# aproposorg/sydr

Measured on AMD Instinct MI355X. Metric: IQ Msamples/s through 32-ch E/P/L correlators @25 MHz fs, higher is better.
Workload: dtype f64

## Files before the change

sydr_amd/csrc/correlator_chip.h:

```cpp
#pragma once

#include "correlator.h"

#pragma clang fp contract(off)

namespace sdr {

constexpr int kChipMax = 26;
constexpr double kChipMinCodeStep = 1.0 / 25.9;
constexpr double kChipMaxCodeStep = 1.0 / 15.5;
constexpr int kChipRawDwords = 13;
constexpr int kChipRotSlots = 2 * kChipMax + 2;
template <int NT>
constexpr int chip_strip_slots() { return 2 * NT + 1; }

__host__ __device__ __forceinline__ int chip_first_above(double thr, double shift, double inv_step, bool& near) {
    const double u = (thr - shift) * inv_step;
    const double fl = floor(u);
    const double fr = u - fl;
    near = near || fr < kNearInteger || fr > 1.0 - kNearInteger;
    return (int)fl + 1;
}
__host__ __device__ __forceinline__ int chip_first_above_exact(int c, double thr, double step, double shift) {
    auto above = [&](int i) {
        double y = (double)i * step;
        y = y + shift;
        return y > thr;
    };
    if (c >= 1 && above(c - 1)) return (c >= 2 && above(c - 2)) ? c - 2 : c - 1;
    if (c < 0) c = 0;
    if (above(c)) return c;
    return above(c + 1) ? c + 1 : c + 2;
}

template <int B, int E, class F>
__device__ __forceinline__ void static_for(F&& f) {
    if constexpr (B < E) {
        f(std::integral_constant<int, B>{});
        static_for<B + 1, E>(f);
    }
}

__device__ __forceinline__ int wave_min_i32(int x) {
#pragma unroll
    for (int off = 1; off < 64; off <<= 1) {
        const int o = __shfl_xor(x, off, 64);
        x = o < x ? o : x;
    }
    return __builtin_amdgcn_readfirstlane(x);
}

#ifndef SDR_BIASED_CVT
#define SDR_BIASED_CVT 1
#endif
constexpr double kCvtBias = 4224.0;
typedef uint32_t sdr_u32x2 __attribute__((ext_vector_type(2)));
__device__ __forceinline__ double biased_sample(sdr_u32x2& pair, uint32_t w_flipped, uint32_t selector, uint32_t hi_const) {
    pair.y = __builtin_amdgcn_perm(w_flipped, hi_const, selector);
    return __builtin_bit_cast(double, pair);
}
constexpr uint32_t cvt_selector(int byte) { return 0x03020000u | ((uint32_t)(4 + byte) << 8) | 0x0Cu; }

template <int NT>
struct ChipGeom {
    int64_t Tfx, Ufx;
    uint64_t delta[NT];
    int q0, F;
    int head_end, tail_start;
    int m[NT], J[NT];
    int bad;
};

template <int NT, int KM, int KS, int KI>
__host__ __device__ __forceinline__ void chip_geometry(int n, const double* shift, const double* step, const double* inv_step,
                                                       ChipGeom<NT>& g) {
    constexpr int A = NT / 2;
    const double two32 = 4294967296.0;
    g.q0 = (int)ceil(shift[A]);
    double y_last = (double)(n - 1) * step[A];
    y_last = y_last + shift[A];
    const int q_last = (int)ceil(y_last);
    g.F = q_last - g.q0 - 1;
    g.head_end = n, g.tail_start = n;
    if (g.F > 0) {
        bool nr = false;
        g.head_end = chip_first_above_exact(chip_first_above((double)g.q0, shift[A], inv_step[A], nr), (double)g.q0, step[A], shift[A]);
        g.tail_start = chip_first_above_exact(chip_first_above((double)(q_last - 1), shift[A], inv_step[A], nr),
                                              (double)(q_last - 1), step[A], shift[A]);
    }
    g.Tfx = (int64_t)rint(inv_step[A] * two32);
    g.Ufx = (int64_t)floor(-shift[A] * inv_step[A] * two32);
    const int M = (int)(g.Tfx >> 32);
    bool bad = M < 1 || M + 1 > kChipMax || g.F > 16384 || (KM != 0 && M != KM);
#pragma unroll
    for (int t = 0; t < NT; ++t) {
        g.m[t] = M, g.J[t] = 0, g.delta[t] = 0;
        if (t == A) continue;
        const int64_t Ut = (int64_t)floor(-shift[t] * inv_step[t] * two32);
        int j = (int)ceil(shift[t] - shift[A]) - 1;
        int64_t d = (Ut - g.Ufx) + (int64_t)(1 + j) * g.Tfx;
        if (d < 0) {
            d += g.Tfx;
            ++j;
        } else if (d >= g.Tfx) {
            d -= g.Tfx;
            --j;
        }
        bad = bad || d < 0 || d >= g.Tfx;
        g.J[t] = j;
        g.delta[t] = (uint64_t)d;
        g.m[t] = (int)(d >> 32);
        bad = bad || (KS != 0 && (g.m[t] != KS || j != (t < A ? -1 : 0)));
        bad = bad || (KI != 0 && !((j == (t - A) * KI - 1 && g.m[t] == 0) || (j == (t - A) * KI && g.m[t] >= M)));
    }
    g.bad = bad ? 1 : 0;
}

constexpr int kStaticHalf = 13;
constexpr int chip_half(int KM, int KS, int KI) { return KI != 0 ? (KM + 2) / 2 : KS + 1; }
struct ChipRot {
    double urc[kStaticHalf + 1], urs[kStaticHalf + 1];
    double rd0c, rd0s, rd1c, rd1s;
    double biasc[3], biass[3];
};
__host__ __device__ inline void chip_rotations(double dphi, int Dmin, ChipRot& r, int half = kStaticHalf, int cmin = kStaticHalf - 2) {
    double cs[16], sn[16];
    for (int k = 0; k < 16; ++k) sincos_reduced(-(double)k * dphi, &sn[k], &cs[k]);
    for (int k = 1; k <= half; ++k) r.urc[k] = cs[k], r.urs[k] = sn[k];
    r.urc[0] = 1.0, r.urs[0] = 0.0;
    sincos_reduced(-(double)Dmin * dphi, &r.rd0s, &r.rd0c);
    sincos_reduced(-(double)(Dmin + 1) * dphi, &r.rd1s, &r.rd1c);
    for (int st = 1; st < 16; st <<= 1)
        for (int l = 15; l >= st; --l) cs[l] += cs[l - st], sn[l] += sn[l - st];
    for (int i = 0; i < 3; ++i) {
        const int l = cmin + i - 1;
        const double re = cs[l] - sn[l], im = cs[l] + sn[l];
        r.biasc[i] = re * 4224.0, r.biass[i] = im * 4224.0;
    }
}

template <int NT>
struct ChipSetup {
    double dphi;
    double shift[NT], step[NT], inv_step[NT];
    int64_t base;
    ChipGeom<NT> g;
    ChipRot r;
};

template <int NT, int KM, int KS, int KI>
__host__ __device__ inline void chip_setup(int n, int64_t start_sample, int64_t capacity, double carrier_hz, double rem_code,
                                           double code_step, const double* spacing, double fs, int stride, ChipSetup<NT>& S) {
    S = ChipSetup<NT>{};
    S.dphi = carrier_step(carrier_hz, fs);
    const double nd = (double)n;
    for (int t = 0; t < NT; ++t) {
        const double shift = rem_code + spacing[t];
        double stop = code_step * nd;
        stop = stop + shift;
        const double delta = stop - shift;
        S.shift[t] = shift;
        S.step[t] = delta / nd;
        S.inv_step[t] = 1.0 / S.step[t];
    }
    const int64_t base = start_sample % capacity;
    const bool applies = code_step >= kChipMinCodeStep && code_step <= kChipMaxCodeStep && base + n + 32 <= capacity;
    S.base = applies ? base : -1;
    if (applies) {
        chip_geometry<NT, KM, KS, KI>(n, S.shift, S.step, S.inv_step, S.g);
        chip_rotations(S.dphi, (int)(((int64_t)stride * S.g.Tfx) >> 32), S.r, chip_half(KM, KS, KI), KM - chip_half(KM, KS, KI));
    }
}

template <int NT>
struct ChipBlock {
    uint32_t raw[kChipRawDwords];
    int S;
    int dn;
    int ds[NT];
};

template <int NT, bool SINGLE_WAVE, int KM = 0, int KS = 0, int KI = 0>
__device__ __forceinline__ bool correlate_epoch_chip(const void* __restrict__ ring, const void* __restrict__ ring_flipped, int64_t capacity,
                                                     const EpochParams& ep, double dphi, const EpochConsts<NT>& K,
                                                     const ChipGeom<NT>& G, int64_t base, const ChipRot* R,
                                                     const uint32_t* lut, double2* strip_lds, double2* rot, int tid,
                                                     int lane, int stride, int edge_lane, double* accr, double* acci) {
    constexpr int A = NT / 2;
    constexpr int kSlots = chip_strip_slots<NT>();
    const int n = ep.n;
    const double* shift = K.shift;
    const double* step = K.step;
    double2* strip = strip_lds + tid * kSlots;
    const int wlane = threadIdx.x & 63;
#pragma unroll
    for (int t = 0; t < NT; ++t) accr[t] = acci[t] = 0.0;

    const double dphi_u = uniform(dphi), rem_carrier_u = uniform(ep.rem_carrier);
    const int q0 = __builtin_amdgcn_readfirstlane(G.q0);
    const int F = __builtin_amdgcn_readfirstlane(G.F);
    const int head_end = __builtin_amdgcn_readfirstlane(G.head_end);
    const int tail_start = __builtin_amdgcn_readfirstlane(G.tail_start);
    (void)ring_flipped;
    const char* ring_base = static_cast<const char*>(ring) + base * 2;

    static_assert(!(KS != 0 && KI != 0), "either the taps switch inside the block (KS) or with it (KI)");
    constexpr bool kStatic = KM != 0 && (KS != 0 || KI != 0);
    constexpr int kHalf = chip_half(KM, KS, KI);
    double urc[kStatic ? kHalf + 1 : 1], urs[kStatic ? kHalf + 1 : 1];
    double biasc[3] = {0.0, 0.0, 0.0}, biass[3] = {0.0, 0.0, 0.0};
    const double two32 = 4294967296.0;
    int64_t Tfx = G.Tfx;
    int64_t stride_fx = (int64_t)stride * Tfx;
    const int Dmin = (int)(stride_fx >> 32);
    if constexpr (kStatic) asm volatile("" : "+v"(Tfx), "+v"(stride_fx));
    double rd0c = 1.0, rd0s = 0.0, rd1c = 1.0, rd1s = 0.0;
    {
        double sn = 0.0, cs = 0.0;
        if constexpr (kStatic) {
            static_assert(kHalf <= kStaticHalf, "the plan's rotations are laid out for half blocks of up to 13 samples");
#pragma unroll
            for (int k = 1; k <= kHalf; ++k) urc[k] = R->urc[k], urs[k] = R->urs[k];
            rd0c = R->rd0c, rd0s = R->rd0s, rd1c = R->rd1c, rd1s = R->rd1s;
            if constexpr (SDR_BIASED_CVT) {
#pragma unroll
                for (int i = 0; i < 3; ++i) biasc[i] = R->biasc[i], biass[i] = R->biass[i];
            }
        } else {
            if (wlane < kChipMax) {
                sincos_reduced(-(double)wlane * dphi_u, &sn, &cs);
                rot[wlane] = make_double2(cs, sn);
            }
            if constexpr (SDR_BIASED_CVT) {
                double br = (cs - sn) * kCvtBias, bi = (cs + sn) * kCvtBias;
#pragma unroll
                for (int off = 1; off < 32; off <<= 1) {
                    const double o_r = __shfl_up(br, off, 64), o_i = __shfl_up(bi, off, 64);
                    br = wlane >= off ? br + o_r : br;
                    bi = wlane >= off ? bi + o_i : bi;
                }
                double2* const btab = rot + kChipMax;
                if (wlane < kChipMax) btab[wlane + 1] = make_double2(br, bi);
                if (wlane == 0) btab[0] = make_double2(0.0, 0.0);
            }
        }
    }

    bool bad = false;
    const int rounds = F > 0 ? (F + stride - 1) / stride : 0;
    if (rounds > 0) {
        int64_t Ufx = G.Ufx;
        const int M = (int)(G.Tfx >> 32);
        if constexpr (kStatic) asm volatile("" : "+v"(Ufx));
        bad = bad || G.bad != 0;
        int m[NT], J[NT];
        uint64_t delta[NT];
        unsigned evmask = (1u << M) | (2u << M);
#pragma unroll
        for (int t = 0; t < NT; ++t) {
            m[t] = G.m[t], J[t] = G.J[t], delta[t] = G.delta[t];
            if constexpr (kStatic) asm volatile("" : "+v"(m[t]), "+v"(J[t]), "+v"(delta[t]));
            if (t != A) evmask |= (1u << m[t]) | (2u << m[t]);
        }
        const int k_last = M + 1;
        int rank[NT];
#pragma unroll
        for (int t = 0; t < NT; ++t) rank[t] = __builtin_popcount(evmask & ((1u << m[t]) - 1u));
        if constexpr (!kStatic) {
            double sn, cs;
            sincos_reduced(-(double)(Dmin + (wlane & 1)) * dphi_u, &sn, &cs);
            rd0c = lane_value(cs, 0), rd0s = lane_value(sn, 0);
            rd1c = lane_value(cs, 1), rd1s = lane_value(sn, 1);
        }
        asm volatile("" : "+v"(rd0c), "+v"(rd0s), "+v"(rd1c), "+v"(rd1s));
        const uint64_t lane_fx = (uint64_t)((int64_t)lane * Tfx);
        uint64_t u_cur = (uint64_t)(Ufx + (int64_t)q0 * Tfx + (int64_t)two32) + lane_fx;
        const int last_idx = F - 1;

        auto prepare = [&](int round, uint64_t u0, ChipBlock<NT>& b) {
            const int idx = round * stride + lane;
            const bool inside = idx <= last_idx;
            const uint64_t uS = inside ? u0 : (uint64_t)(Ufx + (int64_t)(q0 + last_idx) * Tfx + (int64_t)two32);
            const uint64_t uE = uS + (uint64_t)Tfx;
            int S = (int)(uS >> 32);
            int E = (int)(uE >> 32);
            bool near = (uint32_t)uS + 0x10000u < 0x20000u || (uint32_t)uE + 0x10000u < 0x20000u;
            int split[NT];
#pragma unroll
            for (int t = 0; t < NT; ++t) {
                split[t] = 0;
                if (t == A) continue;
                if constexpr (KI != 0) {
                    split[t] = J[t] == (t - A) * KI ? E - S : 0;
                    continue;
                }
                const uint64_t uT = uS + delta[t];
                near = near || (uint32_t)uT + 0x10000u < 0x20000u;
                split[t] = (int)(uT >> 32) - S;
            }
            if (__builtin_expect(__any(near), 0)) {
                const int q = q0 + 1 + (inside ? idx : last_idx);
                S = chip_first_above_exact(S, (double)(q - 1), step[A], shift[A]);
                E = chip_first_above_exact(E, (double)q, step[A], shift[A]);
#pragma unroll
                for (int t = 0; t < NT; ++t) {
                    if (t == A) continue;
                    const int p0 = q + J[t];
                    const int bt = chip_first_above_exact(S + split[t], (double)p0, step[t], shift[t]);
                    double y = (double)S * step[t];
                    y = y + shift[t];
                    const int at_s = (int)ceil(y);
                    bad = bad || (at_s != p0 && at_s != p0 + 1) || (at_s == p0 + 1 && bt > S);
                    split[t] = bt < S ? 0 : bt - S;
                }
            }
            b.S = S;
            const int nn = E - S;
            b.dn = nn - M;
            bad = bad || (unsigned)b.dn > 1u;
#pragma unroll
            for (int t = 0; t < NT; ++t) {
                b.ds[t] = 0;
                if (t == A) continue;
                const int sp = split[t] > nn ? nn : split[t];
                if constexpr (KI != 0) {
                    bad = bad || !(J[t] == (t - A) * KI ? sp == nn : sp == 0);
                    continue;
                }
                b.ds[t] = sp - m[t];
                bad = bad || (unsigned)b.ds[t] > 1u;
            }
            if constexpr (KS != 0 && NT == 3) bad = bad || b.ds[0] != b.ds[2];
            const char* src = ring_base + (int64_t)S * 2;
            const uint4 w0 = *reinterpret_cast<const uint4*>(src);
            const uint4 w1 = *reinterpret_cast<const uint4*>(src + 16);
            const uint4 w2 = *reinterpret_cast<const uint4*>(src + 32);
            const uint32_t w3 = *reinterpret_cast<const uint32_t*>(src + 48);
            b.raw[0] = w0.x, b.raw[1] = w0.y, b.raw[2] = w0.z, b.raw[3] = w0.w;
            b.raw[4] = w1.x, b.raw[5] = w1.y, b.raw[6] = w1.z, b.raw[7] = w1.w;
            b.raw[8] = w2.x, b.raw[9] = w2.y, b.raw[10] = w2.z, b.raw[11] = w2.w;
            b.raw[12] = w3;
        };

        ChipBlock<NT> blk_a, blk_b;
        prepare(0, u_cur, blk_a);
        double sb, cb;
        sincos_reduced(__builtin_fma(-(double)blk_a.S, dphi_u, rem_carrier_u), &sb, &cb);
        if constexpr (!kStatic) {
            sb = lane <= last_idx ? sb : 0.0;
            cb = lane <= last_idx ? cb : 0.0;
        }
        const int q_lane = q0 + 1 + lane + SDR_LUT_PAD;
        const uint32_t* zero_lq = reinterpret_cast<const uint32_t*>(strip) + 3;
        if constexpr (kStatic) strip[0] = strip[1] = make_double2(0.0, 0.0);

        sdr_u32x2 zI = {0u, 0u}, zQ = {0u, 0u};
        asm volatile("" : "+v"(zI), "+v"(zQ));

        auto process = [&](const ChipBlock<NT>& b, int round, double sbk, double cbk) {
            double pr = 0.0, pi = 0.0;
            double2* wp = strip;
            unsigned evm = evmask;
            int klast = k_last;
            if constexpr (!kStatic) asm volatile("" : "+s"(evm), "+s"(klast));
            constexpr int kAhead = 4;
            double2 rr[kChipMax + kAhead];
            if constexpr (!kStatic) {
#pragma unroll
                for (int k = 0; k < kAhead; ++k) rr[k] = rot[k];
            }
            auto park = [&]() {
                *wp = make_double2(pr, pi);
                ++wp;
                asm volatile("" ::: "memory");
            };
            uint32_t hi_rt = 0x40B00000u;
            uint32_t sel_rt[4] = {cvt_selector(0), cvt_selector(1), cvt_selector(2), cvt_selector(3)};
            if constexpr (!kStatic && SDR_BIASED_CVT) {
                asm volatile("" : "+v"(hi_rt));
                asm volatile("" : "+s"(sel_rt[0]), "+s"(sel_rt[1]), "+s"(sel_rt[2]), "+s"(sel_rt[3]));
            }
            auto sample = [&](auto kc) {
                constexpr int k = decltype(kc)::value;
                double ar, ai;
                if constexpr (SDR_BIASED_CVT) {
                    ar = biased_sample(zI, b.raw[k >> 1], sel_rt[(k & 1) ? 2 : 0], hi_rt);
                    ai = biased_sample(zQ, b.raw[k >> 1], sel_rt[(k & 1) ? 3 : 1], hi_rt);
                } else {
                    const int w = ci8_native((int)b.raw[k >> 1]);
                    ar = (k & 1) ? (double)(int)(int8_t)(w >> 16) : (double)(int)(int8_t)w;
                    ai = (k & 1) ? (double)(w >> 24) : (double)(int)(int8_t)(w >> 8);
                }
                if (k + kAhead < kChipMax) rr[k + kAhead] = rot[k + kAhead];
                const double2 r = rr[k];
                pr = __builtin_fma(-ai, r.y, __builtin_fma(ar, r.x, pr));
                pi = __builtin_fma(ai, r.x, __builtin_fma(ar, r.y, pi));
                if constexpr (SDR_BIASED_CVT) asm volatile("" : "+v"(pr), "+v"(pi), "+v"(zI), "+v"(zQ));
            };
            double capr[3] = {0.0, 0.0, 0.0}, capi[3] = {0.0, 0.0, 0.0};
            if constexpr (kStatic) {
                static_assert(2 * kHalf >= KM + 1 && kHalf < KM, "two halves of at most KS + 1 samples cover the block");
                static_assert(!SDR_BIASED_CVT || (2 * kHalf - KM >= 1 && 2 * kHalf - KM <= 2 && (KS == 0 || KS == kHalf - 1)),
                              "the offset's shares are kept for sums of KM - kHalf, + 1 and + 2 samples: kHalf must be one of the last two");
                uint32_t flipped[kChipRawDwords];
                uint32_t hi_const = 0x40B00000u;
                if constexpr (SDR_BIASED_CVT) {
                    asm volatile("" : "+v"(hi_const));
#pragma unroll
                    for (int i = 0; i < kChipRawDwords; ++i) flipped[i] = b.raw[i];
                }
                static_for<0, KM + 1>([&](auto kc) {
                    constexpr int k = decltype(kc)::value;
                    constexpr int j = k < kHalf ? k : k - kHalf;
                    const int w = ci8_native((int)b.raw[k >> 1]);
                    double ar, ai;
                    if constexpr (SDR_BIASED_CVT) {
                        ar = biased_sample(zI, flipped[k >> 1], cvt_selector((k & 1) ? 2 : 0), hi_const);
                        ai = biased_sample(zQ, flipped[k >> 1], cvt_selector((k & 1) ? 3 : 1), hi_const);
                    } else {
                        ar = (k & 1) ? (double)(int)(int8_t)(w >> 16) : (double)(int)(int8_t)w;
                        ai = (k & 1) ? (double)(w >> 24) : (double)(int)(int8_t)(w >> 8);
                    }
                    if constexpr (KS != 0 && k == KS) capr[0] = pr, capi[0] = pi;
                    if constexpr (k == KM) capr[1] = pr, capi[1] = pi;
                    if constexpr (k == kHalf) capr[2] = pr, capi[2] = pi;
                    if constexpr (j == 0) {
                        pr = ar, pi = ai;
                    } else {
                        pr = __builtin_fma(-ai, urs[j], __builtin_fma(ar, urc[j], pr));
                        pi = __builtin_fma(ai, urc[j], __builtin_fma(ar, urs[j], pi));
                    }
                    if constexpr (SDR_BIASED_CVT) asm volatile("" : "+v"(pr), "+v"(pi), "+v"(zI), "+v"(zQ));
                });
            } else if constexpr (KM != 0) {
                static_for<0, KM>([&](auto kc) {
                    constexpr int k = decltype(kc)::value;
                    if (evm & (1u << k)) park();
                    sample(kc);
                });
                park();
                sample(std::integral_constant<int, KM>{});
                park();
            } else {
#pragma unroll
                for (int k = 0; k <= kChipMax; ++k) {
                    if (evm & (1u << k)) {
                        park();
                        if (k == klast) break;
                    }
                    if (k < kChipMax) {
                        double ar, ai;
                        if constexpr (SDR_BIASED_CVT) {
                            ar = biased_sample(zI, b.raw[k >> 1], sel_rt[(k & 1) ? 2 : 0], hi_rt);
                            ai = biased_sample(zQ, b.raw[k >> 1], sel_rt[(k & 1) ? 3 : 1], hi_rt);
                        } else {
                            const int w = ci8_native((int)b.raw[k >> 1]);
                            ar = (k & 1) ? (double)(int)(int8_t)(w >> 16) : (double)(int)(int8_t)w;
                            ai = (k & 1) ? (double)(w >> 24) : (double)(int)(int8_t)(w >> 8);
                        }
                        if (k + kAhead < kChipMax) rr[k + kAhead] = rot[k + kAhead];
                        const double2 r = rr[k];
                        pr = __builtin_fma(-ai, r.y, __builtin_fma(ar, r.x, pr));
                        pi = __builtin_fma(ai, r.x, __builtin_fma(ar, r.y, pi));
                        if constexpr (SDR_BIASED_CVT) asm volatile("" : "+v"(pr), "+v"(pi), "+v"(zI), "+v"(zQ));
                    }
                }
            }
            double2 ptot;
            if constexpr (kStatic && SDR_BIASED_CVT) {
                constexpr int iFirst = 2 * kHalf - KM;
                pr -= biasc[1], pi -= biass[1];
                capr[1] -= biasc[0], capi[1] -= biass[0];
                capr[2] -= biasc[iFirst], capi[2] -= biass[iFirst];
                if constexpr (KS != 0) capr[0] -= biasc[iFirst - 1], capi[0] -= biass[iFirst - 1];
            }
            if constexpr (kStatic) {
                const double qr = b.dn ? pr : capr[1], qi = b.dn ? pi : capi[1];
                ptot.x = __builtin_fma(-qi, urs[kHalf], __builtin_fma(qr, urc[kHalf], capr[2]));
                ptot.y = __builtin_fma(qi, urc[kHalf], __builtin_fma(qr, urs[kHalf], capi[2]));
            } else {
                ptot = strip[rank[A] + b.dn];
                if constexpr (SDR_BIASED_CVT) {
                    const double2 bb = (rot + kChipMax)[M + b.dn];
                    ptot.x -= bb.x, ptot.y -= bb.y;
                }
            }
            const int first = round * stride;
            const uint32_t* lq;
            if constexpr (kStatic)
                lq = first + lane <= last_idx ? lut + q_lane + first : zero_lq;
            else
                lq = lut + q_lane + (first + lane <= last_idx ? first : last_idx - lane);
            if constexpr (KI != 0) {
                const double xr = __builtin_fma(-sbk, ptot.y, cbk * ptot.x);
                const double xi = __builtin_fma(sbk, ptot.x, cbk * ptot.y);
#pragma unroll
                for (int t = 0; t < NT; ++t) {
                    const double c = __hiloint2double((int)lq[(t - A) * KI], 0);
                    accr[t] = __builtin_fma(c, xr, accr[t]);
                    acci[t] = __builtin_fma(c, xi, acci[t]);
                }
                return;
            }
#pragma unroll
            for (int t = 0; t < NT; ++t) {
                double gr, gi;
                if (t == A) {
                    const double c = __hiloint2double((int)lq[0], 0);
                    gr = c * ptot.x;
                    gi = c * ptot.y;
                } else {
                    double2 ps;
                    if constexpr (kStatic)
                        ps = b.ds[NT == 3 ? 0 : t] ? make_double2(capr[2], capi[2]) : make_double2(capr[0], capi[0]);
                    else {
                        ps = strip[rank[t] + b.ds[t]];
                        if constexpr (SDR_BIASED_CVT) {
                            const double2 bb = (rot + kChipMax)[m[t] + b.ds[t]];
                            ps.x -= bb.x, ps.y -= bb.y;
                        }
                    }
                    const int jt = kStatic ? (t < A ? -1 : 0) : J[t];
                    const double ca = __hiloint2double((int)lq[jt], 0);
                    const double cbn = __hiloint2double((int)lq[jt + 1], 0);
                    const double diff = ca - cbn;
                    gr = __builtin_fma(diff, ps.x, cbn * ptot.x);
                    gi = __builtin_fma(diff, ps.y, cbn * ptot.y);
                }
                accr[t] = __builtin_fma(-sbk, gi, __builtin_fma(cbk, gr, accr[t]));
                acci[t] = __builtin_fma(sbk, gr, __builtin_fma(cbk, gi, acci[t]));
            }
        };

        auto wave_has_work = [&](int round) { return SINGLE_WAVE || round * stride + (lane - wlane) <= last_idx; };
        auto advance = [&](const ChipBlock<NT>& from, const ChipBlock<NT>& to, int to_round) {
            const unsigned dd = (unsigned)(to.S - from.S - Dmin);
            const bool alive = to_round * stride + lane <= last_idx;
            bad = bad || (alive && dd > 1u);
            const double rc_ = dd ? rd1c : rd0c, rs_ = dd ? rd1s : rd0s;
            const double cbn = __builtin_fma(cb, rc_, -sb * rs_);
            const double sbn = __builtin_fma(sb, rc_, cb * rs_);
            if constexpr (kStatic) {
                cb = cbn, sb = sbn;
            } else {
                cb = alive ? cbn : 0.0;
                sb = alive ? sbn : 0.0;
            }
        };

        for (int it = 0; it < rounds / 2; ++it) {
            const double sb0 = sb, cb0 = cb;
            u_cur += (uint64_t)stride_fx;
            prepare(2 * it + 1, u_cur, blk_b);
            advance(blk_a, blk_b, 2 * it + 1);
            if (wave_has_work(2 * it)) process(blk_a, 2 * it, sb0, cb0);
            const double sb1 = sb, cb1 = cb;
            if (2 * it + 2 < rounds) {
                u_cur += (uint64_t)stride_fx;
                prepare(2 * it + 2, u_cur, blk_a);
                advance(blk_b, blk_a, 2 * it + 2);
            }
            if (wave_has_work(2 * it + 1)) process(blk_b, 2 * it + 1, sb1, cb1);
        }
        if ((rounds & 1) && wave_has_work(rounds - 1)) process(blk_a, rounds - 1, sb, cb);
    }

    if (__any(bad)) return false;
    if (edge_lane >= 0) {
        if (head_end + (n - tail_start) > 64) {
            for (int off = 0; off < head_end + (n - tail_start); off += 64)
                edge_samples<SDR_FMT_CI8, NT>(ring, capacity, ep, dphi, shift, step, lut, edge_lane + off, head_end, tail_start, accr, acci, base);
        } else {
            edge_samples<SDR_FMT_CI8, NT>(ring, capacity, ep, dphi, shift, step, lut, edge_lane, head_end, tail_start, accr, acci, base);
        }
    }
    return true;
}

__device__ __forceinline__ bool chip_variant_applies(const EpochParams& ep, int64_t capacity) {
    return ep.code_step >= kChipMinCodeStep && ep.code_step <= kChipMaxCodeStep &&
           ep.start_sample % capacity + ep.n + 32 <= capacity;
}

}
```

Before: 96730.

## Track chip block positions with 32-bit fractional walk and derive splits from carries

Replaces the per-block 64-bit fixed-point position arithmetic with a 32-bit fractional walker that advances by the stride and detects boundary crossings via carry bits. In the common case the block length and tap splits are derived directly from carry comparisons, and the exact slow path runs only when some lane is near a boundary. The phase advance now uses the walk carry instead of comparing block starts. It also relaxes a few asm register barriers in the biased conversion path. This cuts integer ALU and register pressure per block but adds ballot and popcount overhead plus more complex consistency checks.

```diff
diff --git a/sydr_amd/csrc/correlator_chip.h b/sydr_amd/csrc/correlator_chip.h
--- a/sydr_amd/csrc/correlator_chip.h
+++ b/sydr_amd/csrc/correlator_chip.h
@@ -114,6 +114,51 @@
         bad = bad || (KI != 0 && !((j == (t - A) * KI - 1 && g.m[t] == 0) || (j == (t - A) * KI && g.m[t] >= M)));
     }
     g.bad = bad ? 1 : 0;
+}
+
+template <int NT>
+struct ChipWalk {
+    uint32_t t_lo, stride_lo, delta_lo[NT];
+    int M, Dmin, m[NT];
+};
+struct ChipWalkPos {
+    int S;
+    uint32_t f;
+};
+template <int NT>
+__host__ __device__ __forceinline__ ChipWalk<NT> chip_walk_make(const ChipGeom<NT>& g, int stride) {
+    ChipWalk<NT> w;
+    const int64_t stride_fx = (int64_t)stride * g.Tfx;
+    w.t_lo = (uint32_t)g.Tfx, w.M = (int)(g.Tfx >> 32);
+    w.stride_lo = (uint32_t)stride_fx, w.Dmin = (int)(stride_fx >> 32);
+#pragma unroll
+    for (int t = 0; t < NT; ++t) w.delta_lo[t] = (uint32_t)g.delta[t], w.m[t] = g.m[t];
+    return w;
+}
+template <int NT>
+__host__ __device__ __forceinline__ ChipWalkPos chip_walk_at(const ChipGeom<NT>& g, int idx) {
+    const uint64_t u = (uint64_t)(g.Ufx + (int64_t)(g.q0 + idx) * g.Tfx + ((int64_t)1 << 32));
+    return ChipWalkPos{(int)(u >> 32), (uint32_t)u};
+}
+__host__ __device__ __forceinline__ bool chip_walk_carry(uint32_t f, uint32_t lo) { return f > ~lo; }
+template <int NT>
+__host__ __device__ __forceinline__ bool chip_walk_step(const ChipWalk<NT>& w, ChipWalkPos& p) {
+    const uint32_t f = p.f + w.stride_lo;
+    const bool c = f < p.f;
+    p.S += w.Dmin + (c ? 1 : 0);
+    p.f = f;
+    return c;
+}
+__host__ __device__ __forceinline__ bool chip_walk_close(uint32_t x) { return x + 0x10000u < 0x20000u; }
+template <int NT, bool SWITCHES>
+__host__ __device__ __forceinline__ bool chip_walk_near(const ChipWalk<NT>& w, uint32_t f) {
+    bool near = chip_walk_close(f) || chip_walk_close(f + w.t_lo);
+    if constexpr (SWITCHES) {
+#pragma unroll
+        for (int t = 0; t < NT; ++t)
+            if (t != NT / 2) near = near || chip_walk_close(f + w.delta_lo[t]);
+    }
+    return near;
 }
 
 constexpr int kStaticHalf = 13;
@@ -176,6 +221,10 @@
 struct ChipBlock {
     uint32_t raw[kChipRawDwords];
     int S;
+    uint32_t f;
+    int exact;
+    int moved;
+    int found;
     int dn;
     int ds[NT];
 };
@@ -209,11 +258,7 @@
     constexpr int kHalf = chip_half(KM, KS, KI);
     double urc[kStatic ? kHalf + 1 : 1], urs[kStatic ? kHalf + 1 : 1];
     double biasc[3] = {0.0, 0.0, 0.0}, biass[3] = {0.0, 0.0, 0.0};
-    const double two32 = 4294967296.0;
-    int64_t Tfx = G.Tfx;
-    int64_t stride_fx = (int64_t)stride * Tfx;
-    const int Dmin = (int)(stride_fx >> 32);
-    if constexpr (kStatic) asm volatile("" : "+v"(Tfx), "+v"(stride_fx));
+    const int Dmin = (int)(((int64_t)stride * G.Tfx) >> 32);
     double rd0c = 1.0, rd0s = 0.0, rd1c = 1.0, rd1s = 0.0;
     {
         double sn = 0.0, cs = 0.0;
@@ -224,7 +269,10 @@
             rd0c = R->rd0c, rd0s = R->rd0s, rd1c = R->rd1c, rd1s = R->rd1s;
             if constexpr (SDR_BIASED_CVT) {
 #pragma unroll
-                for (int i = 0; i < 3; ++i) biasc[i] = R->biasc[i], biass[i] = R->biass[i];
+                for (int i = 0; i < 3; ++i) {
+                    biasc[i] = R->biasc[i], biass[i] = R->biass[i];
+                    if (i == 0) asm volatile("" : "+v"(biasc[i]), "+v"(biass[i]));
+                }
             }
         } else {
             if (wlane < kChipMax) {
@@ -247,19 +295,17 @@
     }
 
     bool bad = false;
+    uint64_t bad_lanes = 0;
     const int rounds = F > 0 ? (F + stride - 1) / stride : 0;
     if (rounds > 0) {
-        int64_t Ufx = G.Ufx;
         const int M = (int)(G.Tfx >> 32);
-        if constexpr (kStatic) asm volatile("" : "+v"(Ufx));
         bad = bad || G.bad != 0;
         int m[NT], J[NT];
-        uint64_t delta[NT];
         unsigned evmask = (1u << M) | (2u << M);
 #pragma unroll
         for (int t = 0; t < NT; ++t) {
-            m[t] = G.m[t], J[t] = G.J[t], delta[t] = G.delta[t];
-            if constexpr (kStatic) asm volatile("" : "+v"(m[t]), "+v"(J[t]), "+v"(delta[t]));
+            m[t] = G.m[t], J[t] = G.J[t];
+            if constexpr (kStatic) asm volatile("" : "+v"(m[t]), "+v"(J[t]));
             if (t != A) evmask |= (1u << m[t]) | (2u << m[t]);
         }
         const int k_last = M + 1;
@@ -273,35 +319,45 @@
             rd1c = lane_value(cs, 1), rd1s = lane_value(sn, 1);
         }
         asm volatile("" : "+v"(rd0c), "+v"(rd0s), "+v"(rd1c), "+v"(rd1s));
-        const uint64_t lane_fx = (uint64_t)((int64_t)lane * Tfx);
-        uint64_t u_cur = (uint64_t)(Ufx + (int64_t)q0 * Tfx + (int64_t)two32) + lane_fx;
+        ChipWalk<NT> W = chip_walk_make(G, stride);
+        if constexpr (kStatic) {
+            asm volatile("" : "+v"(W.t_lo), "+v"(W.stride_lo), "+v"(W.Dmin));
+#pragma unroll
+            for (int t = 0; t < NT; ++t) asm volatile("" : "+v"(W.delta_lo[t]));
+        }
         const int last_idx = F - 1;
-
-        auto prepare = [&](int round, uint64_t u0, ChipBlock<NT>& b) {
+        ChipWalkPos pos = chip_walk_at(G, lane);
+        int last_v = last_idx;
+        asm volatile("" : "+v"(last_v));
+        const ChipWalkPos last_pos = chip_walk_at(G, last_v);
+
+        auto prepare = [&](int round, ChipBlock<NT>& b) {
             const int idx = round * stride + lane;
-            const bool inside = idx <= last_idx;
-            const uint64_t uS = inside ? u0 : (uint64_t)(Ufx + (int64_t)(q0 + last_idx) * Tfx + (int64_t)two32);
-            const uint64_t uE = uS + (uint64_t)Tfx;
-            int S = (int)(uS >> 32);
-            int E = (int)(uE >> 32);
-            bool near = (uint32_t)uS + 0x10000u < 0x20000u || (uint32_t)uE + 0x10000u < 0x20000u;
-            int split[NT];
-#pragma unroll
-            for (int t = 0; t < NT; ++t) {
-                split[t] = 0;
-                if (t == A) continue;
-                if constexpr (KI != 0) {
-                    split[t] = J[t] == (t - A) * KI ? E - S : 0;
-                    continue;
-                }
-                const uint64_t uT = uS + delta[t];
-                near = near || (uint32_t)uT + 0x10000u < 0x20000u;
-                split[t] = (int)(uT >> 32) - S;
-            }
-            if (__builtin_expect(__any(near), 0)) {
+            if (__builtin_expect(round == rounds - 1, 0)) {
+                int i2 = idx;
+                asm volatile("" : "+v"(i2));
+                const bool inside = i2 <= last_idx;
+                pos.S = inside ? pos.S : last_pos.S;
+                pos.f = inside ? pos.f : last_pos.f;
+            }
+            int S = pos.S;
+            const uint32_t f = pos.f;
+            b.exact = (int)__popcll(__ballot(chip_walk_near<NT, KI == 0>(W, f)));
+            if (__builtin_expect(b.exact != 0, 0)) {
+                const bool inside = idx <= last_idx;
                 const int q = q0 + 1 + (inside ? idx : last_idx);
+                int E = S + M + (chip_walk_carry(f, W.t_lo) ? 1 : 0);
+                int split[NT];
+#pragma unroll
+                for (int t = 0; t < NT; ++t) {
+                    split[t] = 0;
+                    if (t == A) continue;
+                    if constexpr (KI != 0) split[t] = J[t] == (t - A) * KI ? E - S : 0;
+                    else split[t] = m[t] + (chip_walk_carry(f, W.delta_lo[t]) ? 1 : 0);
+                }
                 S = chip_first_above_exact(S, (double)(q - 1), step[A], shift[A]);
                 E = chip_first_above_exact(E, (double)q, step[A], shift[A]);
+                b.moved = S - pos.S;
 #pragma unroll
                 for (int t = 0; t < NT; ++t) {
                     if (t == A) continue;
@@ -313,25 +369,38 @@
                     bad = bad || (at_s != p0 && at_s != p0 + 1) || (at_s == p0 + 1 && bt > S);
                     split[t] = bt < S ? 0 : bt - S;
                 }
+                const int nn = E - S;
+                b.dn = nn - M;
+                bad = bad || (unsigned)b.dn > 1u;
+#pragma unroll
+                for (int t = 0; t < NT; ++t) {
+                    b.ds[t] = 0;
+                    if (t == A) continue;
+                    const int sp = split[t] > nn ? nn : split[t];
+                    if constexpr (KI != 0) {
+                        bad = bad || !(J[t] == (t - A) * KI ? sp == nn : sp == 0);
+                        continue;
+                    }
+                    b.ds[t] = sp - m[t];
+                    bad = bad || (unsigned)b.ds[t] > 1u;
+                }
+                if constexpr (KS != 0 && NT == 3) bad = bad || b.ds[0] != b.ds[2];
+                if constexpr (kStatic) {
+                    int found = b.dn | (b.moved << 8);
+#pragma unroll
+                    for (int t = 0; t < NT; ++t) found |= b.ds[t] << (1 + t);
+                    b.found = found;
+                }
+            } else {
+                if constexpr (!kStatic) {
+                    b.dn = chip_walk_carry(f, W.t_lo) ? 1 : 0;
+#pragma unroll
+                    for (int t = 0; t < NT; ++t) b.ds[t] = (t != A && KI == 0 && chip_walk_carry(f, W.delta_lo[t])) ? 1 : 0;
+                }
             }
             b.S = S;
-            const int nn = E - S;
-            b.dn = nn - M;
-            bad = bad || (unsigned)b.dn > 1u;
-#pragma unroll
-            for (int t = 0; t < NT; ++t) {
-                b.ds[t] = 0;
-                if (t == A) continue;
-                const int sp = split[t] > nn ? nn : split[t];
-                if constexpr (KI != 0) {
-                    bad = bad || !(J[t] == (t - A) * KI ? sp == nn : sp == 0);
-                    continue;
-                }
-                b.ds[t] = sp - m[t];
-                bad = bad || (unsigned)b.ds[t] > 1u;
-            }
-            if constexpr (KS != 0 && NT == 3) bad = bad || b.ds[0] != b.ds[2];
-            const char* src = ring_base + (int64_t)S * 2;
+            b.f = f;
+            const char* src = ring_base + (uint32_t)(S * 2);
             const uint4 w0 = *reinterpret_cast<const uint4*>(src);
             const uint4 w1 = *reinterpret_cast<const uint4*>(src + 16);
             const uint4 w2 = *reinterpret_cast<const uint4*>(src + 32);
@@ -343,7 +412,7 @@
         };
 
         ChipBlock<NT> blk_a, blk_b;
-        prepare(0, u_cur, blk_a);
+        prepare(0, blk_a);
         double sb, cb;
         sincos_reduced(__builtin_fma(-(double)blk_a.S, dphi_u, rem_carrier_u), &sb, &cb);
         if constexpr (!kStatic) {
@@ -424,13 +493,16 @@
                     if constexpr (KS != 0 && k == KS) capr[0] = pr, capi[0] = pi;
                     if constexpr (k == KM) capr[1] = pr, capi[1] = pi;
                     if constexpr (k == kHalf) capr[2] = pr, capi[2] = pi;
+                    constexpr bool kCaptured = j != 0 && ((KS != 0 && k == KS) || k == KM);
                     if constexpr (j == 0) {
                         pr = ar, pi = ai;
                     } else {
-                        pr = __builtin_fma(-ai, urs[j], __builtin_fma(ar, urc[j], pr));
-                        pi = __builtin_fma(ai, urc[j], __builtin_fma(ar, urs[j], pi));
+                        const double nr = __builtin_fma(-ai, urs[j], __builtin_fma(ar, urc[j], pr));
+                        const double ni = __builtin_fma(ai, urc[j], __builtin_fma(ar, urs[j], pi));
+                        if constexpr (SDR_BIASED_CVT && kCaptured) asm volatile("" : "+v"(zI), "+v"(zQ) : "v"(nr), "v"(ni));
+                        pr = nr, pi = ni;
                     }
-                    if constexpr (SDR_BIASED_CVT) asm volatile("" : "+v"(pr), "+v"(pi), "+v"(zI), "+v"(zQ));
+                    if constexpr (SDR_BIASED_CVT && !kCaptured) asm volatile("" : "+v"(pr), "+v"(pi), "+v"(zI), "+v"(zQ));
                 });
             } else if constexpr (KM != 0) {
                 static_for<0, KM>([&](auto kc) {
@@ -474,8 +546,22 @@
                 capr[2] -= biasc[iFirst], capi[2] -= biass[iFirst];
                 if constexpr (KS != 0) capr[0] -= biasc[iFirst - 1], capi[0] -= biass[iFirst - 1];
             }
+            bool longer = false, later[NT];
             if constexpr (kStatic) {
-                const double qr = b.dn ? pr : capr[1], qi = b.dn ? pi : capi[1];
+                if (__builtin_expect(b.exact != 0, 0)) {
+                    longer = (b.found & 1) != 0;
+#pragma unroll
+                    for (int t = 0; t < NT; ++t) later[t] = (b.found & (2 << t)) != 0;
+                    asm volatile("" : "+v"(pr));
+                } else {
+                    longer = chip_walk_carry(b.f, W.t_lo);
+#pragma unroll
+                    for (int t = 0; t < NT; ++t) later[t] = chip_walk_carry(b.f, W.delta_lo[t]);
+                    if constexpr (KS != 0 && NT == 3) bad_lanes |= __ballot(later[0]) ^ __ballot(later[2]);
+                }
+            }
+            if constexpr (kStatic) {
+                const double qr = longer ? pr : capr[1], qi = longer ? pi : capi[1];
                 ptot.x = __builtin_fma(-qi, urs[kHalf], __builtin_fma(qr, urc[kHalf], capr[2]));
                 ptot.y = __builtin_fma(qi, urc[kHalf], __builtin_fma(qr, urs[kHalf], capi[2]));
             } else {
@@ -512,7 +598,7 @@
                 } else {
                     double2 ps;
                     if constexpr (kStatic)
-                        ps = b.ds[NT == 3 ? 0 : t] ? make_double2(capr[2], capi[2]) : make_double2(capr[0], capi[0]);
+                        ps = later[NT == 3 ? 0 : t] ? make_double2(capr[2], capi[2]) : make_double2(capr[0], capi[0]);
                     else {
                         ps = strip[rank[t] + b.ds[t]];
                         if constexpr (SDR_BIASED_CVT) {
@@ -533,11 +619,18 @@
         };
 
         auto wave_has_work = [&](int round) { return SINGLE_WAVE || round * stride + (lane - wlane) <= last_idx; };
-        auto advance = [&](const ChipBlock<NT>& from, const ChipBlock<NT>& to, int to_round) {
-            const unsigned dd = (unsigned)(to.S - from.S - Dmin);
-            const bool alive = to_round * stride + lane <= last_idx;
-            bad = bad || (alive && dd > 1u);
-            const double rc_ = dd ? rd1c : rd0c, rs_ = dd ? rd1s : rd0s;
+        auto advance = [&](const ChipBlock<NT>& from, const ChipBlock<NT>& to, int to_round, bool carry) {
+            bool far = carry;
+            if (__builtin_expect((from.exact | to.exact) != 0, 0)) {
+                int idx = to_round * stride + lane;
+                asm volatile("" : "+v"(idx));
+                const auto moved = [&](const ChipBlock<NT>& b) { return !b.exact ? 0 : (kStatic ? b.found >> 8 : b.moved); };
+                const unsigned dd = (unsigned)((carry ? 1 : 0) + moved(to) - moved(from));
+                bad = bad || (idx <= last_idx && dd > 1u);
+                far = dd != 0u;
+            }
+            const bool alive = kStatic || to_round * stride + lane <= last_idx;
+            const double rc_ = far ? rd1c : rd0c, rs_ = far ? rd1s : rd0s;
             const double cbn = __builtin_fma(cb, rc_, -sb * rs_);
             const double sbn = __builtin_fma(sb, rc_, cb * rs_);
             if constexpr (kStatic) {
@@ -550,22 +643,22 @@
 
         for (int it = 0; it < rounds / 2; ++it) {
             const double sb0 = sb, cb0 = cb;
-            u_cur += (uint64_t)stride_fx;
-            prepare(2 * it + 1, u_cur, blk_b);
-            advance(blk_a, blk_b, 2 * it + 1);
+            const bool far_b = chip_walk_step(W, pos);
+            prepare(2 * it + 1, blk_b);
+            advance(blk_a, blk_b, 2 * it + 1, far_b);
             if (wave_has_work(2 * it)) process(blk_a, 2 * it, sb0, cb0);
             const double sb1 = sb, cb1 = cb;
             if (2 * it + 2 < rounds) {
-                u_cur += (uint64_t)stride_fx;
-                prepare(2 * it + 2, u_cur, blk_a);
-                advance(blk_b, blk_a, 2 * it + 2);
+                const bool far_a = chip_walk_step(W, pos);
+                prepare(2 * it + 2, blk_a);
+                advance(blk_b, blk_a, 2 * it + 2, far_a);
             }
             if (wave_has_work(2 * it + 1)) process(blk_b, 2 * it + 1, sb1, cb1);
         }
         if ((rounds & 1) && wave_has_work(rounds - 1)) process(blk_a, rounds - 1, sb, cb);
     }
 
-    if (__any(bad)) return false;
+    if (__any(bad) || bad_lanes != 0) return false;
     if (edge_lane >= 0) {
         if (head_end + (n - tail_start) > 64) {
             for (int off = 0; off < head_end + (n - tail_start); off += 64)
```

Result: no change. 97330 (median of 6 runs) (+0.6%).
